# taaha-khan/2023-CompaCT-Image-Compression

Hardware: AMD Instinct MI355X
Metric: MPixels/s encode+decode, 12-bit 512x512 CT batch, bytes-exact (higher is better)
Workload: dtype u16

## Files before the change

2023-compact-image-compression_amd/csrc/deflate_kernels.hip:

```cpp
#include <hip/hip_runtime.h>
#include <cstring>
#include <algorithm>

#include "cct_internal.h"
#include "../../include/compact_hip.h"

namespace cct {
namespace {

constexpr int MIN_MATCH = 3, MAX_MATCH = 258, WSIZE = 32768;
constexpr int MIN_LOOKAHEAD = MAX_MATCH + MIN_MATCH + 1;
constexpr int MAX_DIST = WSIZE - MIN_LOOKAHEAD;
constexpr int TOO_FAR = 4096;
constexpr int BLOCK_SYMS = 16383;
constexpr int L_CODES = 286, D_CODES = 30, BL_CODES = 19, HEAP_SIZE = 2 * L_CODES + 1;
constexpr int END_BLOCK = 256, MAX_BITS = 15, MAX_BL_BITS = 7;

__constant__ uint8_t c_extra_lbits[29] = {0,0,0,0,0,0,0,0,1,1,1,1,2,2,2,2,3,3,3,3,4,4,4,4,5,5,5,5,0};
__constant__ uint8_t c_extra_dbits[30] = {0,0,0,0,1,1,2,2,3,3,4,4,5,5,6,6,7,7,8,8,9,9,10,10,11,11,12,12,13,13};
__constant__ uint8_t c_extra_blbits[19] = {0,0,0,0,0,0,0,0,0,0,0,0,0,0,0,0,2,3,7};
__constant__ uint8_t c_bl_order[19] = {16,17,18,0,8,7,9,6,10,5,11,4,12,3,13,2,14,1,15};
__constant__ uint8_t c_length_code[256];
__constant__ uint16_t c_base_length[29];
__constant__ uint8_t c_dist_code[512];
// ... 582 lines not shown
	uint32_t ie = base_es[0] + inc_e - ne, is = base_es[1] + inc_s - ns, tot_e = base_es[0];
	for (int w2 = 0; w2 < 4; w2++) {
		const uint32_t te = wsum_e[w2], ts = wsum_s[w2];
		if (w2 < wave) { ie += te; is += ts; }
		tot_e += te;
	}
	if ((uint32_t)tid * 8 < (uint32_t)RUNLEN_OUT && g < L) re[3 * (a.in_stride >> 2) + (g >> 3)] = ie;
#pragma unroll
	for (int k = 0; k < 8; k++) {
		if ((me >> k) & 1u) re[ie++] = g + k + 3;
		if ((ms >> k) & 1u) rs[is++] = g + k;
	}
	if (tid == 0 && c0 + RUNLEN_OUT >= L) a.run_end_count[s] = tot_e;
}

__global__ void __launch_bounds__(256) dfl_run_info_kernel(DeflateArgs a)
{
	const int s = blockIdx.y;
	const uint8_t *in = a.in + (size_t)s * a.in_stride;
	const uint32_t *re = a.run_ends + (size_t)s * a.in_stride;
	const uint32_t *rs = re + (a.in_stride >> 2);
	uint32_t *rl = a.run_ends + (size_t)s * a.in_stride + (a.in_stride >> 1);
	const uint32_t nre = a.run_end_count[s];
	for (uint32_t t = blockIdx.x * blockDim.x + threadIdx.x; t < nre; t += gridDim.x * blockDim.x) {
		const uint32_t x = re[t], len = x - rs[t];
		rl[t] = (len < 511u ? len : 511u) | ((uint32_t)in[x - 1] << 16);
	}
}

__global__ void __launch_bounds__(256) dfl_match_run_kernel(DeflateArgs a, int n)
{
	int s; uint32_t part, nparts;
	if (!xcd_slice(n, s, part, nparts)) return;
	const uint32_t L = a.in_sizes[s];
	const uint8_t *in = a.in + (size_t)s * a.in_stride;
	const size_t base = (size_t)s * a.in_stride;
	const uint64_t *recs = a.rec_out + base;
	uint2 *mr = reinterpret_cast<uint2 *>(a.mr) + base;
	const uint32_t *deep = a.heavy_list + base + a.in_stride - 1;
	const uint32_t ndeep = a.deep_count[s];
	const uint32_t *re = a.run_ends + base;
	const uint32_t *rl = re + (a.in_stride >> 1);
	const uint32_t nre = a.run_end_count[s];
	const uint32_t gen = *a.gen;
	for (uint32_t e = part * blockDim.x + threadIdx.x; e < ndeep; e += nparts * blockDim.x) {
		const uint32_t i = *(deep - e);
		const uint64_t ri = recs[i];
		const uint64_t r_head = recs[i >= 1 ? i - 1 : 0], r_1024 = recs[i >= 1024 ? i - 1024 : 0], r_4096 = recs[i >= 4096 ? i - 4096 : 0];
		const uint32_t p = rec_pos(ri, a.pos_mask);
		const uint32_t h = rec_hash(ri);
		const uint32_t lookahead = L - p;
		const uint32_t max_len = lookahead < (uint32_t)MAX_MATCH ? lookahead : (uint32_t)MAX_MATCH;
		const uint8_t b = in[p], b_prev = in[p >= 1 ? p - 1 : 0];
		const uint32_t r = a.run_len[base + p] & 0x7FFFu;
		const bool has_prev = p >= 2 && b_prev == b;
		uint32_t best4 = has_prev ? r : 0u, q4 = p - 1, best1 = best4, q1 = p - 1;
		bool scan = true;
		if (!has_prev) {
			const uint64_t rh = i >= 1 ? r_head : ~0ull;
			const bool have_head = i >= 1 && rec_hash(rh) == h;
			const uint32_t hq = have_head ? rec_pos(rh, a.pos_mask) : 0u;
			if (!have_head || hq == 0 || hq == nil_candidate(p, lookahead) || p - hq > (uint32_t)MAX_DIST) scan = false;
			else if (p - hq == (uint32_t)MAX_DIST) {
				uint32_t len = 0;
				len = (uint32_t)common_prefix(in + hq, in + p, 0, (int)max_len);
				best4 = best1 = len; q4 = q1 = hq;
				scan = false;
			}
		}
		if (scan && best4 < max_len) {
			const bool ext_ok = r < max_len;
			const uint8_t c = ext_ok ? in[p + r] : 0;
			const uint32_t qw = p >= (uint32_t)MAX_DIST ? p - (uint32_t)MAX_DIST + 1 : 1u;
			uint32_t qmin4 = qw, qmin1 = qw;
			if (i >= 4096 && rec_hash(r_4096) == h) qmin4 = max(qmin4, rec_pos(r_4096, a.pos_mask));
			if (i >= 1024 && rec_hash(r_1024) == h) qmin1 = max(qmin1, rec_pos(r_1024, a.pos_mask));
			uint32_t lo = 0;
			if (p >= 3) {
				lo = re[3 * (a.in_stride >> 2) + ((p - 2) >> 3)];
				while (lo < nre && re[lo] <= p) lo++;
			}
			uint32_t x_n = lo ? re[lo - 1] : 0u, lw_n = lo ? rl[lo - 1] : 0u;
			for (int64_t t = (int64_t)lo - 1; t >= 0; t--) {
				const uint32_t x = x_n;
				const uint32_t lw = lw_n;
				{ const int64_t tn = t > 0 ? t - 1 : 0; x_n = re[tn]; lw_n = rl[tn]; }
				if (x < qmin4 + 3) break;
				if ((lw >> 16) != b) continue;
				const uint32_t m = min(min(lw & 0xFFFFu, r), x - qmin4);
				if (m >= 3) {
					uint32_t q, len;
					if (m == r) {
						q = x - r; len = r;
						if (ext_ok && in[x] == c) len = (uint32_t)common_prefix(in + q, in + p, (int)r + 1, (int)max_len);
					} else { q = x - m; len = m; }
					if (len > best4) { best4 = len; q4 = q; }
					if (x >= qmin1 + 3) {
						const uint32_t m1 = min(m, x - qmin1);
						if (m1 == m) { if (len > best1) { best1 = len; q1 = q; } }
						else if (m1 >= 3 && m1 > best1) { best1 = m1; q1 = x - m1; }
					}
					if (best4 >= max_len) break;
				}
				if (x - m <= qmin4) break;
			}
		}
		mr[p] = pack_match(best4, best1, best4 ? p - q4 : 0u, best1 ? p - q1 : 0u, gen);
	}
}

__device__ __forceinline__ void match_of(const MatchRec &r, uint32_t p, uint32_t npos, int prev_len, int &len, int &dist)
{
	len = 2; dist = 0;
	if (p >= npos || prev_len >= MAX_MATCH) return;
	const int l = prev_len >= 32 ? r.len1024 : r.len4096;
	const int d = prev_len >= 32 ? r.dist1024 : r.dist4096;
	if (l > prev_len && l >= MIN_MATCH) { len = l; dist = d; }
	if (len == MIN_MATCH && dist > TOO_FAR) len = 2;
}
__device__ __forceinline__ void match_at(const MatchRec *mr, const uint16_t *rl, uint32_t gen, uint32_t p, uint32_t npos, int prev_len, int &len, int &dist)
{
	len = 2; dist = 0;
	if (p >= npos || prev_len >= MAX_MATCH) return;
	match_of(checked_match(mr[p], gen, rl[p], p, npos + 2), p, npos, prev_len, len, dist);
}

__global__ void __launch_bounds__(256) dfl_rec_kernel(DeflateArgs a)
{
	const int s = blockIdx.y;
	const uint32_t L = a.in_sizes[s];
	const size_t base = (size_t)s * a.in_stride;
	const uint32_t npos = L >= MIN_MATCH ? L - 2 : 0;
	const MatchRec *mr = reinterpret_cast<const MatchRec *>(a.mr) + base;
	const uint16_t *rl = a.run_len + base;
	const uint32_t nblk64 = (L + 63) / 64;
	const int lane = threadIdx.x & 63;
	const uint32_t gen = *a.gen;
	const uint32_t lastp = npos ? npos - 1 : 0;
	const uint32_t wb_step = gridDim.x * (blockDim.x >> 6);
	struct Req { MatchRec m0, m1; uint32_t w0, w1; };
	auto request = [&](uint32_t wb) {
		const uint32_t p = wb * 64 + lane, pa = min(p, lastp), pb = min(p + 1, lastp);
		return Req{mr[pa], mr[pb], rl[pa], rl[pb]};
	};
	const uint32_t wb0 = blockIdx.x * (blockDim.x >> 6) + (threadIdx.x >> 6);
	Req nx = request(wb0);
	for (uint32_t wb = wb0; wb < nblk64; wb += wb_step) {
		const uint32_t p = wb * 64 + lane;
		const uint32_t blk_end = wb * 64 + 64;
		uint32_t rec = 0, nxt = blk_end, cnt = 0;
		const uint32_t pa = min(p, lastp), pb = min(p + 1, lastp);
		const Req cq = nx;
		nx = request(wb + wb_step);
		const MatchRec r0 = checked_match(cq.m0, gen, cq.w0, pa, L), r1 = checked_match(cq.m1, gen, cq.w1, pb, L);
		if (p < L) {
			int len, dist;
			match_of(r0, p, npos, 2, len, dist);
			if (len < MIN_MATCH) { rec = 0; nxt = p + 1; cnt = 1; }
			else {
				uint32_t k = 0;
				for (;;) {
					int l2, d2;
					if (k == 0) match_of(r1, p + 1, npos, len, l2, d2);
					else match_at(mr, rl, gen, p + k + 1, npos, len, l2, d2);
					if (l2 > len) { len = l2; dist = d2; k++; } else break;
				}
				rec = k | ((uint32_t)len << 8) | ((uint32_t)dist << 17);
				nxt = p + k + (uint32_t)len;
				cnt = k + 1;
			}
		}
		a.rec32[base + p] = rec;
#pragma unroll
		for (int r = 0; r < 6; r++) {
			const bool inside = nxt < blk_end;
			const int j = inside ? (int)(nxt - wb * 64) : lane;
			const uint32_t n2 = __shfl(nxt, j), c2 = __shfl(cnt, j);
			if (inside) { nxt = n2; cnt += c2; }
		}
		a.exit_pos[base + p] = (nxt - blk_end) | (cnt << 16);
	}
}

#ifndef CCT_WALK_T
#define CCT_WALK_T 256
#endif
constexpr int WALK_T = CCT_WALK_T;
__global__ void __launch_bounds__(WALK_T) dfl_walk_kernel(DeflateArgs a, int n)
{
	__shared__ uint32_t s_land[WALK_T];
	__shared__ uint32_t s_wsum[WALK_T / 64];
	const int s = blockIdx.x;
	(void)n;
	const uint32_t L = a.in_sizes[s];
	const size_t base = (size_t)s * a.in_stride;
	const size_t bbase = (size_t)s * (a.in_stride / 64);
	const uint32_t *exit_rec = a.exit_pos + base;
	const int tid = threadIdx.x, lane = tid & 63, wave = tid >> 6;
	const uint32_t seg = (((L + WALK_T - 1) / WALK_T) + 63) & ~63u;
	const uint32_t seg_end = min(L, (uint32_t)(tid + 1) * seg);
	uint32_t start = min(L, (uint32_t)tid * seg), land = start, cnt = 0;
	auto hop_through = [&]() {
		uint32_t cur = start, c = 0;
		while (cur < seg_end) { const uint32_t e = exit_rec[cur]; c += e >> 16; cur = (cur & ~63u) + 64u + (e & 0xFFFFu); }
		land = cur; cnt = c;
	};
	hop_through();
	for (;;) {
		__syncthreads();
		s_land[tid] = land;
		__syncthreads();
		const uint32_t pl = tid ? s_land[tid - 1] : 0u;
		const bool moved = tid > 0 && pl != start;
		if (!__syncthreads_or(moved)) break;
		if (moved) { start = pl; hop_through(); }
	}
	uint32_t inc = cnt;
#pragma unroll
	for (int d = 1; d < 64; d <<= 1) { const uint32_t o = __shfl_up(inc, d, 64); if (lane >= d) inc += o; }
	if (lane == 63) s_wsum[wave] = inc;
	__syncthreads();
	uint32_t syms = inc - cnt;
	for (int w = 0; w < wave; w++) syms += s_wsum[w];
	if (tid == WALK_T - 1) a.total_syms[s] = syms + cnt;
	for (uint32_t cur = start; cur < seg_end;) {
		const uint32_t b = cur >> 6;
		a.blk_entry[bbase + b] = cur;
		a.blk_symbase[bbase + b] = syms;
		const uint32_t e = exit_rec[cur];
		syms += e >> 16;
		cur = (cur & ~63u) + 64u + (e & 0xFFFFu);
	}
}

__global__ void __launch_bounds__(256) dfl_symbols_kernel(DeflateArgs a)
{
	const int s = blockIdx.y;
	const uint32_t L = a.in_sizes[s];
	const uint8_t *in = a.in + (size_t)s * a.in_stride;
	const size_t base = (size_t)s * a.in_stride;
	const size_t bbase = (size_t)s * (a.in_stride / 64);
	const uint32_t nblk64 = (L + 63) / 64;
	const int lane = threadIdx.x & 63;
	uint32_t *sym = a.sym + base;
	uint32_t *bend = a.blk_end + (size_t)s * a.max_blocks;
	const uint32_t wb_step = gridDim.x * (blockDim.x >> 6), wb_last = nblk64 ? nblk64 - 1 : 0;
	struct Req { uint32_t entry, symbase, rec; uint8_t lit0; };
	auto request = [&](uint32_t wb) {
		const uint32_t wbc = min(wb, wb_last), pc = min(wbc * 64 + lane, L - 1);
		return Req{a.blk_entry[bbase + wbc], a.blk_symbase[bbase + wbc], a.rec32[base + pc], in[pc]};
	};
	const uint32_t wb0 = blockIdx.x * (blockDim.x >> 6) + (threadIdx.x >> 6);
	Req nx = nblk64 ? request(wb0) : Req{0xFFFFFFFFu, 0, 0, 0};
	for (uint32_t wb = wb0; wb < nblk64; wb += wb_step) {
		const uint32_t p = wb * 64 + lane;
		const Req cur_req = nx;
		nx = request(wb + wb_step);
		const uint32_t entry = cur_req.entry, symbase = cur_req.symbase;
		uint32_t rec = cur_req.rec;
		const uint8_t lit0 = cur_req.lit0;
		if (entry == 0xFFFFFFFFu) continue;
		if (p >= L) rec = 0;
		const uint32_t k = rec & 0xFFu, len = (rec >> 8) & 0x1FFu, dist = rec >> 17;
		const uint32_t nxt = len ? p + k + len : p + 1;
		const uint32_t cnt = len ? k + 1 : 1;
		const uint64_t jump = __ballot(len != 0);
		const uint32_t nvalid = min(64u, L - wb * 64);
		uint64_t visited = 0;
		uint32_t cur = (uint32_t)__builtin_amdgcn_readfirstlane((int)(entry - wb * 64));
		while (cur < nvalid) {
			const uint64_t rest = jump >> cur;
			if (!rest) { visited |= ~0ull << cur; break; }
			const int d = __ffsll((long long)rest) - 1;
			visited |= (d >= 63 ? ~0ull : ((2ull << d) - 1ull)) << cur;
			cur = (uint32_t)__builtin_amdgcn_readlane((int)nxt, (int)cur + d) - wb * 64;
		}
		if (nvalid < 64) visited &= (1ull << nvalid) - 1ull;
		const bool mine = (visited >> lane) & 1ull;
		uint32_t v = mine ? cnt : 0u, inc = v;
#pragma unroll
		for (int d = 1; d < 64; d <<= 1) {
			const uint32_t t = __shfl_up(inc, d);
			if (lane >= d) inc += t;
		}
		uint32_t off = symbase + inc - v;
		if (mine) {
			if (p == L - 1) a.postloop_lit[s] = 1;
			for (uint32_t t = 0; t < (len ? k : 1u); t++, off++) {
				sym[off] = t ? in[p + t] : lit0;
				if (off % BLOCK_SYMS == BLOCK_SYMS - 1) bend[off / BLOCK_SYMS] = p + t + 1;
			}
			if (len) {
				sym[off] = (len - MIN_MATCH) | (dist << 16);
				if (off % BLOCK_SYMS == BLOCK_SYMS - 1) bend[off / BLOCK_SYMS] = p + k + len;
			}
		}
	}
}

struct TreeScratch {
	uint16_t freq[HEAP_SIZE], dad[HEAP_SIZE], len[HEAP_SIZE], code[L_CODES + 2];
	uint16_t dfreq[2 * D_CODES + 1], ddad[2 * D_CODES + 1], dlen[2 * D_CODES + 1], dcode[D_CODES + 2];
	uint16_t bfreq[2 * BL_CODES + 1], bdad[2 * BL_CODES + 1], blen[2 * BL_CODES + 1], bcode[BL_CODES + 1];
	alignas(16) uint32_t heap[HEAP_SIZE + 3];
	uint32_t bl_count[MAX_BITS + 1];
	uint16_t next_code[MAX_BITS + 1];
	int heap_len, heap_max, max_code, overflow, lmax, dmax;
	uint32_t opt_len, static_len, dyn_body_bits;
	uint32_t hdr_bits[160];
	uint32_t hdr_nbits;
	int ntok, btype, max_blindex;
	uint8_t extra_l[29], extra_d[30], extra_bl[19], bl_order[19];
	__device__ __forceinline__ uint32_t *hist_l() { return heap; }
	__device__ __forceinline__ uint32_t *hist_d() { return heap + L_CODES + 2; }
	__device__ __forceinline__ uint8_t *length_code() { return reinterpret_cast<uint8_t *>(dad); }
	__device__ __forceinline__ uint8_t *dist_code() { return reinterpret_cast<uint8_t *>(dad) + 256; }
	__device__ __forceinline__ uint16_t *tok() { return dad; }
};
static_assert(sizeof(TreeScratch) <= 8192, "13 tree waves per CU: keep the working set around 8 KB");
static_assert(HEAP_SIZE >= L_CODES + D_CODES, "token list fits dad[]");
static_assert((HEAP_SIZE + 1) * 4 >= (L_CODES + 2 + D_CODES) * 4 && HEAP_SIZE * 2 >= 768, "aliases fit");
__device__ __forceinline__ uint32_t static_llen(int n) { return n <= 143 ? 8u : n <= 255 ? 9u : n <= 279 ? 7u : 8u; }

typedef __attribute__((address_space(3))) uint16_t lds_u16;
struct TreeView { lds_u16 *freq, *dad, *len, *code; };

__device__ __forceinline__ uint32_t uni(uint32_t x) { return (uint32_t)__builtin_amdgcn_readfirstlane((int)x); }
__device__ __forceinline__ void pqdownheap(TreeScratch &S, int k, int hl)
{
	const uint32_t v = uni(S.heap[k]);
	const uint32_t vk = v >> 10;
	int j = k << 1;
	while (j <= hl) {
		uint2 pr = *reinterpret_cast<const uint2 *>(&S.heap[j]);
		uint4 gc = *reinterpret_cast<const uint4 *>(&S.heap[min(2 * j, (HEAP_SIZE & ~3))]);
		pr.x = uni(pr.x); pr.y = uni(pr.y);
		gc.x = uni(gc.x); gc.y = uni(gc.y); gc.z = uni(gc.z); gc.w = uni(gc.w);
		uint32_t e = pr.x;
		int c = j;
		if (j < hl && (pr.y >> 10) <= (pr.x >> 10)) { c = j + 1; e = pr.y; }
		if (vk <= (e >> 10)) break;
		S.heap[k] = e;
		k = c;
		j = c << 1;
		if (j > hl) break;
		const bool left = (c & 1) == 0;
		const uint32_t x2 = left ? gc.x : gc.z, y2 = left ? gc.y : gc.w;
		e = x2;
		c = j;
		if (j < hl && (y2 >> 10) <= (x2 >> 10)) { c = j + 1; e = y2; }
		if (vk <= (e >> 10)) break;
		S.heap[k] = e;
		k = c;
		j = c << 1;
	}
	S.heap[k] = v;
}

__device__ __forceinline__ uint32_t sift_root(TreeScratch &S, uint32_t v, int hl, int levels)
{
	if (levels == 0) { S.heap[1] = v; return v; }
	const uint2 p0 = *reinterpret_cast<const uint2 *>(&S.heap[2]);
	uint32_t right = (2 < hl && p0.y <= (p0.x | 1023u)) ? 1u : 0u;
	uint32_t e = right ? p0.y : p0.x;
	uint32_t moving = v > (e | 1023u) ? 1u : 0u;
	const uint32_t rootv = moving ? e : v;
	S.heap[1] = rootv;
	uint32_t k = 2u + right;
	for (int l = 1; l < levels - 1; l++) {
		const uint32_t j = k << 1;
		const uint2 pr = *reinterpret_cast<const uint2 *>(&S.heap[j]);
		right = pr.y <= (pr.x | 1023u) ? 1u : 0u;
		e = right ? pr.y : pr.x;
		const uint32_t go = (moving && v > (e | 1023u)) ? 1u : 0u;
		S.heap[moving ? k : 0u] = go ? e : v;
		k = go ? j + right : k;
		moving = go;
	}
	if (levels >= 2) {
		const uint32_t j = k << 1;
		const uint2 pr = *reinterpret_cast<const uint2 *>(&S.heap[min(j, (uint32_t)(HEAP_SIZE - 1))]);
		right = (j < (uint32_t)hl && pr.y <= (pr.x | 1023u)) ? 1u : 0u;
		e = right ? pr.y : pr.x;
		const uint32_t go = (moving && j <= (uint32_t)hl && v > (e | 1023u)) ? 1u : 0u;
		S.heap[moving ? k : 0u] = go ? e : v;
		k = go ? j + right : k;
		moving = go;
	}
	S.heap[moving ? k : 0u] = v;
	return rootv;
}


__device__ __forceinline__ TreeView view_of(TreeScratch &S, int kind)
{
	if (kind == 0) return TreeView{(lds_u16 *)S.freq, (lds_u16 *)S.dad, (lds_u16 *)S.len, (lds_u16 *)S.code};
	if (kind == 1) return TreeView{(lds_u16 *)S.dfreq, (lds_u16 *)S.ddad, (lds_u16 *)S.dlen, (lds_u16 *)S.dcode};
	return TreeView{(lds_u16 *)S.bfreq, (lds_u16 *)S.bdad, (lds_u16 *)S.blen, (lds_u16 *)S.bcode};
}
__device__ __forceinline__ int elems_of(int kind) { return kind == 0 ? L_CODES : kind == 1 ? D_CODES : BL_CODES; }

__device__ void tree_leaves(TreeScratch &S, int kind)
{
	const TreeView t = view_of(S, kind);
	const int lane = threadIdx.x, elems = elems_of(kind);
	const uint64_t lt_mask = (1ull << lane) - 1ull;
	int max_code = -1;
	uint32_t nleaf = 0;
	for (int n0 = 0; n0 < elems; n0 += 64) {
		const int n = n0 + lane;
		const uint32_t f = n < elems ? t.freq[n] : 0u;
		const uint64_t bal = __ballot(f != 0);
		if (f != 0) S.heap[1 + nleaf + (uint32_t)__popcll(bal & lt_mask)] = (f << 15) | (uint32_t)n;
		else if (n < elems) t.len[n] = 0;
		if (bal) max_code = n0 + 63 - __clzll((long long)bal);
		nleaf += (uint32_t)__popcll(bal);
	}
	if (lane == 0) { S.heap_len = (int)nleaf; S.max_code = max_code; }
}

__device__ void tree_heap(TreeScratch &S, int kind)
{
	const TreeView t = view_of(S, kind);
	int n, m, node, max_code = (int)uni((uint32_t)S.max_code);
	int heap_len = (int)uni((uint32_t)S.heap_len), heap_max = HEAP_SIZE;
	while (heap_len < 2) {
		node = max_code < 2 ? ++max_code : 0;
		t.freq[node] = 1; S.opt_len--;
		S.heap[++heap_len] = (1u << 15) | (uint32_t)node;
		if (kind == 0) S.static_len -= static_llen(node);
		else if (kind == 1) S.static_len -= 5;
	}
	for (n = heap_len / 2; n >= 1; n--) pqdownheap(S, n, heap_len);
	node = elems_of(kind);
	uint32_t top = S.heap[1];
	do {
		const uint32_t en = top;
		const uint32_t lastv = S.heap[heap_len];
		heap_len--;
		const int levels = 31 - __clz(heap_len | 1);
		const uint32_t em = sift_root(S, lastv, heap_len, levels);
		n = (int)(en & 1023u); m = (int)(em & 1023u);
		S.heap[--heap_max] = en; S.heap[--heap_max] = em;
		const uint32_t f = (en >> 15) + (em >> 15);
		const uint32_t dn = (en >> 10) & 31u, dm = (em >> 10) & 31u;
		const uint32_t d = (dn >= dm ? dn : dm) + 1;
		t.freq[node] = (uint16_t)f;
		t.dad[n] = t.dad[m] = (uint16_t)node;
		top = sift_root(S, (f << 15) | (d << 10) | (uint32_t)node, heap_len, levels);
		node++;
	} while (heap_len >= 2);
	S.heap[--heap_max] = top;
	S.heap_len = heap_len; S.heap_max = heap_max;
	S.max_code = max_code;
}

__device__ void tree_depths(TreeScratch &S, int kind)
{
	const TreeView t = view_of(S, kind);
	const int lane = threadIdx.x;
	const int max_length = kind == 2 ? MAX_BL_BITS : MAX_BITS;
	const int base = kind == 0 ? 257 : 0;
	const int max_code = S.max_code, heap_max = S.heap_max;
	const uint32_t root = S.heap[heap_max];
	constexpr uint16_t UNKNOWN = 0xFFFF;
	for (int h = heap_max + 1 + lane; h < HEAP_SIZE; h += 64) t.len[S.heap[h] & 1023u] = UNKNOWN;
	if (lane == 0) t.len[root & 1023u] = 0;
	if (lane <= MAX_BITS) S.bl_count[lane] = 0;
	__syncthreads();
	for (bool again = true; again;) {
		again = false;
		for (int h0 = heap_max + 1; h0 < HEAP_SIZE; h0 += 64) {
			const int h = h0 + lane;
			bool unknown = false;
			if (h < HEAP_SIZE) {
				const int n = (int)(S.heap[h] & 1023u);
				if (t.len[n] == UNKNOWN) {
					const uint32_t ld = t.len[t.dad[n]];
					if (ld == UNKNOWN) unknown = true;
					else t.len[n] = (uint16_t)min(ld + 1u, (uint32_t)max_length);
				}
			}
			if (__ballot(unknown)) again = true;
		}
		__syncthreads();
	}
	int overflow = 0;
	for (int h0 = heap_max + 1; h0 < HEAP_SIZE; h0 += 64) {
		const int h = h0 + lane;
		const bool clamped = h < HEAP_SIZE && t.len[t.dad[S.heap[h] & 1023u]] == (uint32_t)max_length;
		overflow += (int)__popcll(__ballot(clamped));
	}
	uint32_t o = 0, st = 0;
	for (int n = lane; n <= max_code; n += 64) {
		const uint32_t f = t.freq[n];
		if (f == 0) continue;
		const uint32_t bits = t.len[n];
		atomicAdd(&S.bl_count[bits], 1u);
		uint32_t xbits = 0;
		if (n >= base) xbits = kind == 0 ? S.extra_l[n - base] : kind == 1 ? S.extra_d[n] : S.extra_bl[n];
		o += f * (bits + xbits);
		if (kind == 0) st += f * (static_llen(n) + xbits);
		else if (kind == 1) st += f * (5u + xbits);
	}
	o = wave_sum(o); st = wave_sum(st);
	if (lane == 0) { S.overflow = overflow; S.opt_len += o; S.static_len += st; }
}

__device__ void tree_fix(TreeScratch &S, int kind)
{
	const TreeView t = view_of(S, kind);
	const int max_length = kind == 2 ? MAX_BL_BITS : MAX_BITS;
	const int max_code = S.max_code;
	int overflow = S.overflow;
	if (overflow > 0) {
		int bits, n, m, h = HEAP_SIZE;
		do {
			bits = max_length - 1;
			while (S.bl_count[bits] == 0) bits--;
			S.bl_count[bits]--; S.bl_count[bits + 1] += 2; S.bl_count[max_length]--;
			overflow -= 2;
		} while (overflow > 0);
		for (bits = max_length; bits != 0; bits--) {
			n = (int)S.bl_count[bits];
			while (n != 0) {
				m = (int)(S.heap[--h] & 1023u);
				if (m > max_code) continue;
				if ((uint32_t)t.len[m] != (uint32_t)bits) {
					S.opt_len += ((uint32_t)bits - t.len[m]) * t.freq[m];
					t.len[m] = (uint16_t)bits;
				}
				n--;
			}
		}
	}
	uint32_t code = 0;
	for (int bits = 1; bits <= MAX_BITS; bits++) { code = (code + S.bl_count[bits - 1]) << 1; S.next_code[bits] = (uint16_t)code; }
}

__device__ void tree_codes(TreeScratch &S, int kind)
{
	const TreeView t = view_of(S, kind);
	const int lane = threadIdx.x, max_code = S.max_code;
	const uint64_t lt_mask = (1ull << lane) - 1ull;
	uint32_t seen[MAX_BITS + 1];
#pragma unroll
	for (int b = 1; b <= MAX_BITS; b++) seen[b] = S.next_code[b];
	for (int n0 = 0; n0 <= max_code; n0 += 64) {
		const int n = n0 + lane;
		const int len = n <= max_code ? (int)t.len[n] : 0;
		uint32_t mine = 0;
#pragma unroll
		for (int b = 1; b <= MAX_BITS; b++) {
			const uint64_t bal = __ballot(len == b);
			if (len == b) mine = seen[b] + (uint32_t)__popcll(bal & lt_mask);
			seen[b] += (uint32_t)__popcll(bal);
		}
		if (len != 0) t.code[n] = (uint16_t)(__brev(mine) >> (32 - len));
	}
}

__device__ void scan_tree_wave(TreeScratch &S, const TreeView &t, int max_code)
{
	const int lane = threadIdx.x;
	constexpr int NCH = (L_CODES + 63) / 64;
	const int n_el = max_code + 1;
	uint32_t v[NCH];
	uint64_t startmask[NCH];
#pragma unroll
	for (int c = 0; c < NCH; c++) {
		const int n = c * 64 + lane;
		v[c] = n < n_el ? (uint32_t)t.len[n] : 0xFFFFu;
		const uint32_t before = n == 0 ? 0xFFFFFFFFu : (uint32_t)t.len[max(n - 1, 0)];
		startmask[c] = __ballot(n < n_el && v[c] != before);
	}
	uint16_t *tk = S.tok();
	uint32_t base = (uint32_t)S.ntok;
#pragma unroll
	for (int c = 0; c < NCH; c++) {
		if (c * 64 >= n_el) break;
		const int n = c * 64 + lane;
		const bool start = (startmask[c] >> lane) & 1ull;
		uint32_t R = 0;
		if (start) {
			int nxt = n_el;
			const uint64_t rest = lane < 63 ? startmask[c] >> (lane + 1) : 0ull;
			if (rest) nxt = n + (int)__ffsll((long long)rest);
			else {
#pragma unroll
				for (int c2 = NCH - 1; c2 > c; c2--) if (startmask[c2]) nxt = min(nxt, c2 * 64 + (int)__ffsll((long long)startmask[c2]) - 1);
			}
			R = (uint32_t)(nxt - n);
		}
		const uint32_t val = v[c];
		uint32_t nlit_head = 0, nrep6 = 0, tail_lit = 0, tail_sym = 0xFFFFFFFFu, nbig = 0;
		if (start) {
			if (val != 0) {
				if (R < 4) nlit_head = R;
				else if (R <= 6) { nlit_head = 1; tail_sym = 16u | ((R - 4u) << 5); }
				else {
					nlit_head = 1; nrep6 = 1 + (R - 7u) / 6u;
					const uint32_t r = (R - 7u) % 6u;
					if (r < 3) tail_lit = r; else tail_sym = 16u | ((r - 3u) << 5);
				}
			} else {
				nbig = R / 138u;
				const uint32_t r = R % 138u;
				if (r < 3) tail_lit = r;
				else if (r <= 10) tail_sym = 17u | ((r - 3u) << 5);
				else tail_sym = 18u | ((r - 11u) << 5);
			}
		}
		const uint32_t ntok = nlit_head + nrep6 + nbig + tail_lit + (tail_sym != 0xFFFFFFFFu ? 1u : 0u);
		uint32_t inc = ntok;
#pragma unroll
		for (int d = 1; d < 64; d <<= 1) { const uint32_t o = (uint32_t)__shfl_up((int)inc, d, 64); if (lane >= d) inc += o; }
		if (start) {
			uint32_t w = base + inc - ntok;
			for (uint32_t i = 0; i < nlit_head; i++) tk[w++] = (uint16_t)val;
			for (uint32_t i = 0; i < nrep6; i++) tk[w++] = (uint16_t)(16u | (3u << 5));
			for (uint32_t i = 0; i < nbig; i++) tk[w++] = (uint16_t)(18u | (127u << 5));
			for (uint32_t i = 0; i < tail_lit; i++) tk[w++] = (uint16_t)val;
			if (tail_sym != 0xFFFFFFFFu) tk[w++] = (uint16_t)tail_sym;
			if (nlit_head + tail_lit) atomicAdd(&S.hdr_bits[val], nlit_head + tail_lit);
			if (nrep6) atomicAdd(&S.hdr_bits[16], nrep6);
			if (nbig) atomicAdd(&S.hdr_bits[18], nbig);
			if (tail_sym != 0xFFFFFFFFu) atomicAdd(&S.hdr_bits[tail_sym & 31u], 1u);
		}
		base += (uint32_t)__shfl((int)inc, 63, 64);
	}
	if (lane == 0) S.ntok = (int)base;
}

__device__ __forceinline__ void hdr_or(TreeScratch &S, uint32_t pos, uint32_t value, uint32_t n)
{
	const uint32_t w = pos >> 5, sh = pos & 31u;
	atomicOr(&S.hdr_bits[w], value << sh);
	if (sh + n > 32u) atomicOr(&S.hdr_bits[w + 1], value >> (32u - sh));
}

__device__ void send_header(TreeScratch &S)
{
	const int lane = threadIdx.x;
	const int nbl = S.max_blindex + 1;
	if (lane == 0) hdr_or(S, 0, (uint32_t)(S.lmax + 1 - 257) | ((uint32_t)(S.dmax + 1 - 1) << 5) | ((uint32_t)(nbl - 4) << 10), 14);
	if (lane < nbl) hdr_or(S, 14u + 3u * (uint32_t)lane, S.blen[S.bl_order[lane]], 3);
	uint32_t base = 14u + 3u * (uint32_t)nbl;
	const uint16_t *tk = S.tok();
	const int nt = S.ntok;
	for (int c0 = 0; c0 < nt; c0 += 64) {
		const int i = c0 + lane;
		uint32_t nbits = 0, val = 0;
		if (i < nt) {
			const uint32_t sym = tk[i] & 31u, ex = tk[i] >> 5;
			const uint32_t cl = S.blen[sym];
			nbits = cl + S.extra_bl[sym];
			val = (uint32_t)S.bcode[sym] | (ex << cl);
		}
		uint32_t inc = nbits;
#pragma unroll
		for (int d = 1; d < 64; d <<= 1) { const uint32_t o = (uint32_t)__shfl_up((int)inc, d, 64); if (lane >= d) inc += o; }
		if (nbits) hdr_or(S, base + inc - nbits, val, nbits);
		base += (uint32_t)__shfl((int)inc, 63, 64);
	}
	if (lane == 0) S.hdr_nbits = base;
}

constexpr int TREE_BLOCKS = 1;
__global__ void __launch_bounds__(64) dfl_tree_kernel(DeflateArgs a)
{
	__shared__ TreeScratch S4[TREE_BLOCKS];
	const int s = blockIdx.y, m0 = blockIdx.x * TREE_BLOCKS, lane = threadIdx.x;
	const uint32_t T = a.total_syms[s];
	const uint32_t L = a.in_sizes[s];
	uint32_t nfull = T / BLOCK_SYMS;
	if (T % BLOCK_SYMS == 0 && nfull > 0 && a.postloop_lit[s]) nfull--;
	const uint32_t nblocks = nfull + 1;
	BlockMeta *meta = a.block_meta + (size_t)s * a.max_blocks;
	if ((uint32_t)m0 >= nblocks) return;
	const int nb = (int)min((uint32_t)TREE_BLOCKS, nblocks - (uint32_t)m0);
	const uint32_t *bend = a.blk_end + (size_t)s * a.max_blocks;
	const bool owner = lane < nb;
#ifdef CCT_TREE_PROF
	long long tp[16]; int tpi = 0;
#define TREE_STAMP() do { if (tpi < 16) tp[tpi++] = clock64(); } while (0)
#else
#define TREE_STAMP() do {} while (0)
#endif
	TREE_STAMP();

	for (int q = 0; q < nb; q++) {
		TreeScratch &S = S4[q];
		const int m = m0 + q;
		const bool last = (uint32_t)m == nblocks - 1;
		const uint32_t first = (uint32_t)m * BLOCK_SYMS;
		const uint32_t nsym = last ? T - first : (uint32_t)BLOCK_SYMS;
		const uint32_t *sym = a.sym + (size_t)s * a.in_stride + first;
		for (int i = lane; i < HEAP_SIZE; i += 64) { S.freq[i] = 0; S.len[i] = 0; }
		for (int i = lane; i < L_CODES + 2; i += 64) S.code[i] = 0;
		for (int i = lane; i < 2 * D_CODES + 1; i += 64) { S.dfreq[i] = 0; S.dlen[i] = 0; S.ddad[i] = 0; }
		for (int i = lane; i < D_CODES + 2; i += 64) S.dcode[i] = 0;
		for (int i = lane; i < 2 * BL_CODES + 1; i += 64) { S.bfreq[i] = 0; S.blen[i] = 0; S.bdad[i] = 0; }
		for (int i = lane; i < BL_CODES + 1; i += 64) S.bcode[i] = 0;
		uint8_t *length_code = S.length_code(), *dist_code = S.dist_code();
		{
			uint8_t dc[8], lc4[4];
#pragma unroll
			for (int k = 0; k < 8; k++) dc[k] = c_dist_code[lane + 64 * k];
#pragma unroll
			for (int k = 0; k < 4; k++) lc4[k] = c_length_code[lane + 64 * k];
			const int l29 = min(lane, 28), l30 = min(lane, 29), l19 = min(lane, 18);
			const uint8_t xl = c_extra_lbits[l29], xd = c_extra_dbits[l30], xb = c_extra_blbits[l19], bo = c_bl_order[l19];
#pragma unroll
			for (int k = 0; k < 8; k++) dist_code[lane + 64 * k] = dc[k];
#pragma unroll
			for (int k = 0; k < 4; k++) length_code[lane + 64 * k] = lc4[k];
			if (lane < 29) S.extra_l[lane] = xl;
			if (lane < 30) S.extra_d[lane] = xd;
			if (lane < 19) { S.extra_bl[lane] = xb; S.bl_order[lane] = bo; }
		}
		uint32_t *hl = S.hist_l(), *hd = S.hist_d();
		for (int i = lane; i < L_CODES; i += 64) hl[i] = 0;
		if (lane < D_CODES) hd[lane] = 0;
		__syncthreads();
		{
			const uint32_t lasts = nsym ? nsym - 1 : 0;
			uint32_t nv[16];
#pragma unroll
			for (int k = 0; k < 16; k++) nv[k] = sym[min((uint32_t)(k * 64 + lane), lasts)];
			for (uint32_t i0 = 0; i0 < nsym; i0 += 64 * 16) {
				uint32_t v[16];
#pragma unroll
				for (int k = 0; k < 16; k++) v[k] = nv[k];
#pragma unroll
				for (int k = 0; k < 16; k++) nv[k] = sym[min(i0 + 1024u + (uint32_t)(k * 64 + lane), lasts)];
#pragma unroll
				for (int k = 0; k < 16; k++) {
					if (i0 + (uint32_t)(k * 64 + lane) >= nsym) continue;
					const uint32_t dist = v[k] >> 16, lc = v[k] & 0xFFu;
					if (dist == 0) atomicAdd(&hl[lc], 1u);
					else {
						const uint32_t d1 = dist - 1;
						atomicAdd(&hl[length_code[lc] + 256 + 1], 1u);
						atomicAdd(&hd[d1 < 256 ? dist_code[d1] : dist_code[256 + (d1 >> 7)]], 1u);
					}
				}
			}
		}
		__syncthreads();
		for (int i = lane; i < L_CODES; i += 64) S.freq[i] = (uint16_t)hl[i];
		if (lane < D_CODES) S.dfreq[lane] = (uint16_t)hd[lane];
		for (int i = lane; i < 160; i += 64) S.hdr_bits[i] = 0;
		if (lane == 0) { S.opt_len = 0; S.static_len = 0; S.hdr_nbits = 0; S.ntok = 0; S.btype = 0; S.max_blindex = 0; }
		__syncthreads();
		if (lane == 0) S.freq[END_BLOCK] = 1;
		for (int i = lane; i < HEAP_SIZE; i += 64) S.dad[i] = 0;
	}
	__syncthreads();
	TREE_STAMP();
#pragma unroll 1
	for (int kind = 0; kind < 3; kind++) {
		if (kind == 2) {
			if (owner) S4[lane].dyn_body_bits = S4[lane].opt_len;
			__syncthreads();
			for (int q = 0; q < nb; q++) {
				TreeScratch &S = S4[q];
				scan_tree_wave(S, view_of(S, 0), S.lmax);
				__syncthreads();
				scan_tree_wave(S, view_of(S, 1), S.dmax);
				__syncthreads();
				if (lane < BL_CODES) { S.bfreq[lane] = (uint16_t)S.hdr_bits[lane]; S.hdr_bits[lane] = 0; }
			}
			__syncthreads();
		}
		for (int q = 0; q < nb; q++) tree_leaves(S4[q], kind);
		__syncthreads();
		TREE_STAMP();
		if (owner) tree_heap(S4[lane], kind);
		__syncthreads();
		TREE_STAMP();
		for (int q = 0; q < nb; q++) tree_depths(S4[q], kind);
		__syncthreads();
		if (owner) {
			tree_fix(S4[lane], kind);
			if (kind == 0) S4[lane].lmax = S4[lane].max_code; else if (kind == 1) S4[lane].dmax = S4[lane].max_code;
		}
		__syncthreads();
		for (int q = 0; q < nb; q++) tree_codes(S4[q], kind);
		__syncthreads();
		TREE_STAMP();
	}
	if (owner) {
		TreeScratch &S = S4[lane];
		const int m = m0 + lane;
		const bool last = (uint32_t)m == nblocks - 1;
		const uint32_t first = (uint32_t)m * BLOCK_SYMS;
		const uint32_t nsym = last ? T - first : (uint32_t)BLOCK_SYMS;
		const uint32_t in_begin = m == 0 ? 0u : bend[m - 1];
		const uint32_t in_end = last ? L : bend[m];
		int max_blindex;
		for (max_blindex = BL_CODES - 1; max_blindex >= 3; max_blindex--)
			if (S.blen[S.bl_order[max_blindex]] != 0) break;
		S.opt_len += 3 * ((uint32_t)max_blindex + 1) + 5 + 5 + 4;
		uint32_t opt_lenb = (S.opt_len + 3 + 7) >> 3;
		const uint32_t static_lenb = (S.static_len + 3 + 7) >> 3;
		if (static_lenb <= opt_lenb) opt_lenb = static_lenb;
		const uint32_t stored_len = in_end - in_begin;
		BlockMeta bm;
		bm.in_begin = in_begin; bm.stored_len = stored_len; bm.first_sym = first; bm.nsym = nsym; bm.last = last ? 1u : 0u;
		if (stored_len + 4 <= opt_lenb) {
			bm.type = 0; bm.hdr_nbits = 0; bm.body_bits = 0;
		} else if (static_lenb == opt_lenb) {
			bm.type = 1; bm.hdr_nbits = 0; bm.body_bits = S.static_len;
		} else {
			bm.type = 2; bm.hdr_nbits = 0;
			bm.body_bits = S.dyn_body_bits;
		}
		S.btype = (int)bm.type; S.max_blindex = max_blindex;
		meta[m] = bm;
		if (m == 0) a.n_blocks[s] = nblocks;
	}
	__syncthreads();
	for (int q = 0; q < nb; q++) {
		TreeScratch &S = S4[q];
		if (S.btype != 2) continue;
		send_header(S);
		__syncthreads();
		BlockTables *bt = a.block_tables + ((size_t)s * a.max_blocks + m0 + q);
		for (int i = lane; i * 32 < (int)S.hdr_nbits; i += 64) bt->hdr_bits[i] = S.hdr_bits[i];
		if (lane == 0) meta[m0 + q].hdr_nbits = S.hdr_nbits;
	}
	__syncthreads();
	TREE_STAMP();
#ifdef CCT_TREE_PROF
	if (s == 0 && m0 == 0 && lane == 0) {
		printf("[tree prof] nb=%d:", nb);
		for (int i = 1; i < tpi; i++) printf(" %lld", tp[i] - tp[i - 1]);
		printf("  (hist | leaves0 heap0 rest0 | scan+leaves1 heap1 rest1 | scan_tree+leaves2 heap2 rest2 | final)\n");
	}
#endif
	for (int q = 0; q < nb; q++) {
		TreeScratch &S = S4[q];
		BlockTables *bt = a.block_tables + ((size_t)s * a.max_blocks + m0 + q);
		for (int i = lane; i < L_CODES; i += 64) { bt->lcode[i] = S.code[i]; bt->llen[i] = (uint8_t)S.len[i]; }
		if (lane < D_CODES) { bt->dcode[lane] = S.dcode[lane]; bt->dlen[lane] = (uint8_t)S.dlen[lane]; }
	}
}

__global__ void __launch_bounds__(256) dfl_adler_kernel(DeflateArgs a)
{
	__shared__ unsigned long long sa[256], sb[256];
	const int s = blockIdx.x;
	const uint32_t L = a.in_sizes[s];
	const uint8_t *in = a.in + (size_t)s * a.in_stride;
	unsigned long long A = 0, B = 0;
	const uint32_t nfull = L / 16;
	constexpr int U = 8;
	for (uint32_t g0 = threadIdx.x; g0 < nfull; g0 += blockDim.x * U) {
		uint4 v[U];
#pragma unroll
		for (int u = 0; u < U; u++) v[u] = *reinterpret_cast<const uint4 *>(in + (size_t)min(g0 + (uint32_t)u * blockDim.x, nfull - 1) * 16);
#pragma unroll
		for (int u = 0; u < U; u++) {
			const uint32_t g = g0 + (uint32_t)u * blockDim.x;
			if (g >= nfull) continue;
			const uint32_t w[4] = {v[u].x, v[u].y, v[u].z, v[u].w};
			uint32_t sd = 0, sk = 0;
#pragma unroll
			for (int k = 0; k < 16; k++) { const uint32_t d = (w[k >> 2] >> ((k & 3) * 8)) & 0xFFu; sd += d; sk += (uint32_t)k * d; }
			A += sd;
			B += (unsigned long long)(L - g * 16) * sd - sk;
		}
	}
	if (threadIdx.x == 0)
		for (uint32_t i = nfull * 16; i < L; i++) { const unsigned long long d = in[i]; A += d; B += (unsigned long long)(L - i) * d; }
	sa[threadIdx.x] = A; sb[threadIdx.x] = B;
	__syncthreads();
	for (int st = 128; st > 0; st >>= 1) {
		if ((int)threadIdx.x < st) { sa[threadIdx.x] += sa[threadIdx.x + st]; sb[threadIdx.x] += sb[threadIdx.x + st]; }
		__syncthreads();
	}
	if (threadIdx.x == 0) {
		const uint32_t lo = (uint32_t)((1ull + sa[0]) % 65521ull);
		const uint32_t hi = (uint32_t)(((unsigned long long)L + sb[0]) % 65521ull);
		a.adler[s] = (hi << 16) | lo;
	}
}

__global__ void dfl_layout_kernel(DeflateArgs a, int n)
{
	const int s = blockIdx.x * blockDim.x + threadIdx.x;
	if (s >= n) return;
	uint8_t *out = a.out + (size_t)s * a.out_stride;
	for (int i = 0; i < 13; i++) out[i] = a.header13[i];
	out[13] = 0x78; out[14] = 0xDA;
	uint64_t bit = 8ull * 15;
	BlockMeta *meta = a.block_meta + (size_t)s * a.max_blocks;
	const uint32_t nb = a.n_blocks[s];
	for (uint32_t m = 0; m < nb; m++) {
		BlockMeta bm = meta[m];
		bm.bit_off = bit;
		if (bm.type == 0) {
			bit = (bit + 3 + 7) & ~7ull;
			bit += 32 + 8ull * bm.stored_len;
		} else {
			bit += 3 + bm.hdr_nbits + bm.body_bits;
		}
		if (bm.last) bit = (bit + 7) & ~7ull;
		meta[m] = bm;
	}
	const uint64_t byte = bit >> 3;
	const uint32_t ad = a.adler[s];
	out[byte + 0] = (uint8_t)(ad >> 24); out[byte + 1] = (uint8_t)(ad >> 16);
	out[byte + 2] = (uint8_t)(ad >> 8);  out[byte + 3] = (uint8_t)ad;
	a.out_sizes[s] = (uint32_t)(byte + 4);
}

__device__ __forceinline__ void or_bits(uint32_t *words, uint64_t bit, uint64_t value, int nbits)
{
	if (nbits == 0) return;
	const uint64_t w = bit >> 5;
	const int sh = (int)(bit & 31);
	const uint64_t lo = value << sh;
	const uint64_t hi = sh ? (value >> (64 - sh)) : 0ull;
	atomicOr(&words[w], (uint32_t)lo);
	if (sh + nbits > 32) atomicOr(&words[w + 1], (uint32_t)(lo >> 32));
	if (sh + nbits > 64) atomicOr(&words[w + 2], (uint32_t)hi);
}

__global__ void __launch_bounds__(256) dfl_emit_kernel(DeflateArgs a)
{
	__shared__ uint32_t wsum[4];
	__shared__ unsigned long long s_run;
	const int s = blockIdx.y, m = blockIdx.x;
	if ((uint32_t)m >= a.n_blocks[s]) return;
	const BlockMeta bm = a.block_meta[(size_t)s * a.max_blocks + m];
	const BlockTables *bt = a.block_tables + ((size_t)s * a.max_blocks + m);
	uint8_t *out = a.out + (size_t)s * a.out_stride;
	uint32_t *words = reinterpret_cast<uint32_t *>(out);
	const uint8_t *in = a.in + (size_t)s * a.in_stride;
	uint64_t bit = bm.bit_off;
	if (bm.type == 0) {
		if (threadIdx.x == 0) or_bits(words, bit, (uint64_t)bm.last, 3);
		const uint64_t byte = ((bit + 3 + 7) & ~7ull) >> 3;
		if (threadIdx.x == 0) {
			out[byte] = (uint8_t)(bm.stored_len & 0xFF); out[byte + 1] = (uint8_t)(bm.stored_len >> 8);
			out[byte + 2] = (uint8_t)(~bm.stored_len & 0xFF); out[byte + 3] = (uint8_t)((~bm.stored_len >> 8) & 0xFF);
		}
		for (uint32_t i = threadIdx.x; i < bm.stored_len; i += blockDim.x) out[byte + 4 + i] = in[bm.in_begin + i];
		return;
	}
	if (threadIdx.x == 0) or_bits(words, bit, (uint64_t)((bm.type << 1) + bm.last), 3);
	bit += 3;
	if (bm.type == 2) {
		for (uint32_t i = threadIdx.x; i * 32 < bm.hdr_nbits; i += blockDim.x) {
			const int nb = (int)min(32u, bm.hdr_nbits - i * 32);
			or_bits(words, bit + 32ull * i, bt->hdr_bits[i], nb);
		}
		bit += bm.hdr_nbits;
	}
	const uint32_t *sym = a.sym + (size_t)s * a.in_stride + bm.first_sym;
	const bool dyn = bm.type == 2;
	const int lane = threadIdx.x & 63, wave = threadIdx.x >> 6;
	__shared__ uint16_t t_lcode[L_CODES + 2], t_dcode[D_CODES + 2];
	__shared__ uint8_t t_llen[L_CODES + 2], t_dlen[D_CODES + 2];
	__shared__ uint32_t wbuf[400];
	__shared__ uint8_t t_length_code[256], t_dist_code[512], t_extra_l[32], t_extra_d[32];
	__shared__ uint16_t t_base_length[32], t_base_dist[32];
	{
		const int t = threadIdx.x, t2 = min(t + 256, L_CODES - 1), td = min(t, D_CODES - 1), t29 = min(t, 28), t30 = min(t, 29);
		const uint16_t *lsrc = dyn ? bt->lcode : c_static_lcode, *dsrc = dyn ? bt->dcode : c_static_dcode;
		const uint8_t *llsrc = dyn ? bt->llen : c_static_llen;
		const uint16_t lc0 = lsrc[t], lc1 = lsrc[t2];
		const uint8_t ll0 = llsrc[t], ll1 = llsrc[t2];
		const uint16_t dc = dsrc[td];
		uint8_t dl = bt->dlen[td];
		if (!dyn) dl = 5;
		const uint8_t k0 = c_dist_code[t], k1 = c_dist_code[t + 256], lcd = c_length_code[t];
		const uint8_t xl = c_extra_lbits[t29], xd = c_extra_dbits[t30];
		const uint16_t bl = c_base_length[t29], bd = c_base_dist[t30];
		t_lcode[t] = lc0; t_llen[t] = ll0;
		if (t + 256 < L_CODES) { t_lcode[t + 256] = lc1; t_llen[t + 256] = ll1; }
		if (t < D_CODES) { t_dcode[t] = dc; t_dlen[t] = dl; }
		t_dist_code[t] = k0; t_dist_code[t + 256] = k1; t_length_code[t] = lcd;
		if (t < 29) { t_extra_l[t] = xl; t_base_length[t] = bl; }
		if (t < 30) { t_extra_d[t] = xd; t_base_dist[t] = bd; }
	}
	if (threadIdx.x == 0) s_run = bit;
	for (int i = threadIdx.x; i < 400; i += blockDim.x) wbuf[i] = 0;
	__syncthreads();
	const uint32_t last_sym = bm.nsym ? bm.nsym - 1 : 0;
	uint32_t vnext = sym[min((uint32_t)threadIdx.x, last_sym)];
	for (uint32_t base = 0; base <= bm.nsym; base += blockDim.x) {
		const uint32_t i = base + threadIdx.x;
		uint64_t bits = 0;
		int nb = 0;
		const uint32_t v = vnext;
		vnext = sym[min(i + blockDim.x, last_sym)];
		if (i < bm.nsym) {
			uint32_t dist = v >> 16;
			const uint32_t lc = v & 0xFFu;
			if (dist == 0) {
				bits = t_lcode[lc];
				nb = t_llen[lc];
			} else {
				int code = t_length_code[lc];
				const int lsym = code + 256 + 1;
				bits = t_lcode[lsym];
				nb = t_llen[lsym];
				int extra = t_extra_l[code];
				if (extra) { bits |= (uint64_t)(lc - t_base_length[code]) << nb; nb += extra; }
				dist--;
				code = dist < 256 ? t_dist_code[dist] : t_dist_code[256 + (dist >> 7)];
				bits |= (uint64_t)t_dcode[code] << nb;
				nb += t_dlen[code];
				extra = t_extra_d[code];
				if (extra) { bits |= (uint64_t)(dist - t_base_dist[code]) << nb; nb += extra; }
			}
		} else if (i == bm.nsym) {
			bits = t_lcode[END_BLOCK];
			nb = t_llen[END_BLOCK];
		}
		uint32_t inc = (uint32_t)nb;
#pragma unroll
		for (int d = 1; d < 64; d <<= 1) {
			const uint32_t t = __shfl_up(inc, d);
			if (lane >= d) inc += t;
		}
		if (lane == 63) wsum[wave] = inc;
		__syncthreads();
		uint32_t wb = 0, tot = 0;
		for (int w = 0; w < 4; w++) { if (w < wave) wb += wsum[w]; tot += wsum[w]; }
		const uint64_t run = s_run;
		const uint32_t lbit = (uint32_t)(run & 31) + wb + inc - (uint32_t)nb;
		if (nb) {
			const uint32_t w0 = lbit >> 5, sh = lbit & 31;
			const uint64_t lo = bits << sh;
			atomicOr(&wbuf[w0], (uint32_t)lo);
			if (sh + nb > 32) atomicOr(&wbuf[w0 + 1], (uint32_t)(lo >> 32));
			if (sh + nb > 64) atomicOr(&wbuf[w0 + 2], (uint32_t)(bits >> (64 - sh)));
		}
		__syncthreads();
		const uint32_t nwords = ((uint32_t)(run & 31) + tot + 31) >> 5;
		const uint64_t gw = run >> 5;
		for (uint32_t k = threadIdx.x; k < nwords; k += blockDim.x) {
			const uint32_t v = wbuf[k];
			if (v) atomicOr(&words[gw + k], v);
			wbuf[k] = 0;
		}
		if (threadIdx.x == 0) s_run = run + tot;
		__syncthreads();
	}
}

__global__ void __launch_bounds__(256) dfl_pack_offsets_kernel(const uint32_t *sizes, int n, uint64_t *offsets, int exact)
{
	if (threadIdx.x == 0 && blockIdx.x == 0) {
		uint64_t acc = 0;
		for (int i = 0; i < n; i++) { offsets[i] = acc; acc += exact ? sizes[i] : ((sizes[i] + 15u) & ~15u); }
		offsets[n] = acc;
	}
}
__global__ void __launch_bounds__(256) dfl_pack_kernel(const uint8_t *src, size_t stride, const uint32_t *sizes,
                                                       const uint64_t *offsets, uint8_t *dst)
{
	const int s = blockIdx.y;
	const uint32_t n16 = (sizes[s] + 15u) >> 4;
	const uint4 *in = reinterpret_cast<const uint4 *>(src + (size_t)s * stride);
	uint4 *out = reinterpret_cast<uint4 *>(dst + offsets[s]);
	for (uint32_t i = blockIdx.x * blockDim.x + threadIdx.x; i < n16; i += gridDim.x * blockDim.x) out[i] = in[i];
}

__global__ void dfl_offsets2_kernel(DeflateArgs a, int n)
{
	const size_t per = a.in_stride / 64;
	for (size_t i = blockIdx.x * (size_t)blockDim.x + threadIdx.x; i < (size_t)n * per; i += (size_t)gridDim.x * blockDim.x)
		a.blk_entry[i] = 0xFFFFFFFFu;
}

__global__ void dfl_offsets_kernel(DeflateArgs a, int n)
{
// ... 129 lines not shown
```

Before: 15470.

## Pipeline Huffman heap sifts across wave lanes instead of one lane per block

Huffman tree construction changes from one lane handling a whole block to a whole wave cooperating on each block in turn. Heapify now runs level by level with lanes sifting nodes in parallel, and the extract/merge loop keeps up to eight sift-downs in flight on separate lanes. Each sift advances one level per tick and a ballot checks for conflicts before the next pop. This targets the long serial dependency chain of the heap loop, but blocks are now processed one after another rather than one per lane, and the lane-synchronised ticking adds overhead and correctness risk.

Result: faster. 16240 (median of 6 runs) (+5.0%).

```diff
diff --git a/2023-compact-image-compression_amd/csrc/deflate_kernels.hip b/2023-compact-image-compression_amd/csrc/deflate_kernels.hip
--- a/2023-compact-image-compression_amd/csrc/deflate_kernels.hip
+++ b/2023-compact-image-compression_amd/csrc/deflate_kernels.hip
@@ -908,7 +908,7 @@
 	uint16_t freq[HEAP_SIZE], dad[HEAP_SIZE], len[HEAP_SIZE], code[L_CODES + 2];
 	uint16_t dfreq[2 * D_CODES + 1], ddad[2 * D_CODES + 1], dlen[2 * D_CODES + 1], dcode[D_CODES + 2];
 	uint16_t bfreq[2 * BL_CODES + 1], bdad[2 * BL_CODES + 1], blen[2 * BL_CODES + 1], bcode[BL_CODES + 1];
-	alignas(16) uint32_t heap[HEAP_SIZE + 3];
+	alignas(16) uint32_t heap[HEAP_SIZE + 11];
 	uint32_t bl_count[MAX_BITS + 1];
 	uint16_t next_code[MAX_BITS + 1];
 	int heap_len, heap_max, max_code, overflow, lmax, dmax;
@@ -931,72 +931,19 @@
 typedef __attribute__((address_space(3))) uint16_t lds_u16;
 struct TreeView { lds_u16 *freq, *dad, *len, *code; };
 
-__device__ __forceinline__ uint32_t uni(uint32_t x) { return (uint32_t)__builtin_amdgcn_readfirstlane((int)x); }
 __device__ __forceinline__ void pqdownheap(TreeScratch &S, int k, int hl)
 {
-	const uint32_t v = uni(S.heap[k]);
-	const uint32_t vk = v >> 10;
-	int j = k << 1;
-	while (j <= hl) {
-		uint2 pr = *reinterpret_cast<const uint2 *>(&S.heap[j]);
-		uint4 gc = *reinterpret_cast<const uint4 *>(&S.heap[min(2 * j, (HEAP_SIZE & ~3))]);
-		pr.x = uni(pr.x); pr.y = uni(pr.y);
-		gc.x = uni(gc.x); gc.y = uni(gc.y); gc.z = uni(gc.z); gc.w = uni(gc.w);
-		uint32_t e = pr.x;
-		int c = j;
-		if (j < hl && (pr.y >> 10) <= (pr.x >> 10)) { c = j + 1; e = pr.y; }
-		if (vk <= (e >> 10)) break;
+	const uint32_t v = S.heap[k];
+	for (int j = k << 1; j <= hl; j = k << 1) {
+		const uint2 pr = *reinterpret_cast<const uint2 *>(&S.heap[j]);
+		const int right = (j < hl && pr.y <= (pr.x | 1023u)) ? 1 : 0;
+		const uint32_t e = right ? pr.y : pr.x;
+		if (v <= (e | 1023u)) break;
 		S.heap[k] = e;
-		k = c;
-		j = c << 1;
-		if (j > hl) break;
-		const bool left = (c & 1) == 0;
-		const uint32_t x2 = left ? gc.x : gc.z, y2 = left ? gc.y : gc.w;
-		e = x2;
-		c = j;
-		if (j < hl && (y2 >> 10) <= (x2 >> 10)) { c = j + 1; e = y2; }
-		if (vk <= (e >> 10)) break;
-		S.heap[k] = e;
-		k = c;
-		j = c << 1;
+		k = j + right;
 	}
 	S.heap[k] = v;
 }
-
-__device__ __forceinline__ uint32_t sift_root(TreeScratch &S, uint32_t v, int hl, int levels)
-{
-	if (levels == 0) { S.heap[1] = v; return v; }
-	const uint2 p0 = *reinterpret_cast<const uint2 *>(&S.heap[2]);
-	uint32_t right = (2 < hl && p0.y <= (p0.x | 1023u)) ? 1u : 0u;
-	uint32_t e = right ? p0.y : p0.x;
-	uint32_t moving = v > (e | 1023u) ? 1u : 0u;
-	const uint32_t rootv = moving ? e : v;
-	S.heap[1] = rootv;
-	uint32_t k = 2u + right;
-	for (int l = 1; l < levels - 1; l++) {
-		const uint32_t j = k << 1;
-		const uint2 pr = *reinterpret_cast<const uint2 *>(&S.heap[j]);
-		right = pr.y <= (pr.x | 1023u) ? 1u : 0u;
-		e = right ? pr.y : pr.x;
-		const uint32_t go = (moving && v > (e | 1023u)) ? 1u : 0u;
-		S.heap[moving ? k : 0u] = go ? e : v;
-		k = go ? j + right : k;
-		moving = go;
-	}
-	if (levels >= 2) {
-		const uint32_t j = k << 1;
-		const uint2 pr = *reinterpret_cast<const uint2 *>(&S.heap[min(j, (uint32_t)(HEAP_SIZE - 1))]);
-		right = (j < (uint32_t)hl && pr.y <= (pr.x | 1023u)) ? 1u : 0u;
-		e = right ? pr.y : pr.x;
-		const uint32_t go = (moving && j <= (uint32_t)hl && v > (e | 1023u)) ? 1u : 0u;
-		S.heap[moving ? k : 0u] = go ? e : v;
-		k = go ? j + right : k;
-		moving = go;
-	}
-	S.heap[moving ? k : 0u] = v;
-	return rootv;
-}
-
 
 __device__ __forceinline__ TreeView view_of(TreeScratch &S, int kind)
 {
@@ -1025,40 +972,86 @@
 	if (lane == 0) { S.heap_len = (int)nleaf; S.max_code = max_code; }
 }
 
+constexpr int TREE_SIFTS = 8;
 __device__ void tree_heap(TreeScratch &S, int kind)
 {
 	const TreeView t = view_of(S, kind);
-	int n, m, node, max_code = (int)uni((uint32_t)S.max_code);
-	int heap_len = (int)uni((uint32_t)S.heap_len), heap_max = HEAP_SIZE;
-	while (heap_len < 2) {
-		node = max_code < 2 ? ++max_code : 0;
-		t.freq[node] = 1; S.opt_len--;
-		S.heap[++heap_len] = (1u << 15) | (uint32_t)node;
-		if (kind == 0) S.static_len -= static_llen(node);
-		else if (kind == 1) S.static_len -= 5;
-	}
-	for (n = heap_len / 2; n >= 1; n--) pqdownheap(S, n, heap_len);
-	node = elems_of(kind);
-	uint32_t top = S.heap[1];
-	do {
-		const uint32_t en = top;
-		const uint32_t lastv = S.heap[heap_len];
-		heap_len--;
-		const int levels = 31 - __clz(heap_len | 1);
-		const uint32_t em = sift_root(S, lastv, heap_len, levels);
-		n = (int)(en & 1023u); m = (int)(em & 1023u);
-		S.heap[--heap_max] = en; S.heap[--heap_max] = em;
-		const uint32_t f = (en >> 15) + (em >> 15);
-		const uint32_t dn = (en >> 10) & 31u, dm = (em >> 10) & 31u;
-		const uint32_t d = (dn >= dm ? dn : dm) + 1;
-		t.freq[node] = (uint16_t)f;
-		t.dad[n] = t.dad[m] = (uint16_t)node;
-		top = sift_root(S, (f << 15) | (d << 10) | (uint32_t)node, heap_len, levels);
-		node++;
-	} while (heap_len >= 2);
-	S.heap[--heap_max] = top;
-	S.heap_len = heap_len; S.heap_max = heap_max;
-	S.max_code = max_code;
+	const int lane = threadIdx.x;
+	int max_code = S.max_code, h = S.heap_len;
+	while (h < 2) {
+		const int node = max_code < 2 ? ++max_code : 0;
+		h++;
+		if (lane == 0) {
+			t.freq[node] = 1; S.opt_len--;
+			S.heap[h] = (1u << 15) | (uint32_t)node;
+			if (kind == 0) S.static_len -= static_llen(node);
+			else if (kind == 1) S.static_len -= 5;
+		}
+	}
+	__syncthreads();
+	for (int d = 31 - __clz(h >> 1); d >= 0; d--) {
+		const int lo = 1 << d, hi = min((2 << d) - 1, h >> 1);
+		for (int n0 = lo; n0 <= hi; n0 += 64) {
+			if (n0 + lane <= hi) pqdownheap(S, n0 + lane, h);
+			__builtin_amdgcn_wave_barrier();
+		}
+	}
+	if (lane < TREE_SIFTS) {
+		uint32_t v = 0, k = 1, hl = 0, w = 0;
+		bool moving = false;
+		const uint32_t sink = HEAP_SIZE + 3 + lane;
+		auto tick = [&]() {
+			const uint32_t j = k << 1;
+			const uint2 pr = *reinterpret_cast<const uint2 *>(&S.heap[j]);
+			const uint32_t right = (j < hl && pr.y <= (pr.x | 1023u)) ? 1u : 0u;
+			const uint32_t e = right ? pr.y : pr.x;
+			const bool go = moving && j <= hl && v > (e | 1023u);
+			w = go ? e : v;
+			uint32_t at = moving ? k : sink;
+			asm volatile("" : "+v"(at), "+v"(w));
+			S.heap[at] = w;
+			k = go ? j + right : k;
+			moving = go;
+			__builtin_amdgcn_wave_barrier();
+		};
+		auto start = [&](int slot, uint32_t x) {
+			const bool me = lane == slot;
+			v = me ? x : v; k = me ? 1u : k; hl = me ? (uint32_t)h : hl; moving = moving || me;
+		};
+		int node = elems_of(kind), hm = HEAP_SIZE, slot = 0;
+		uint32_t en = S.heap[1];
+		for (;;) {
+			while (__ballot(moving && ((uint32_t)h >> (__clz(k | 1u) - __clz(h))) == k)) tick();
+			h--;
+			start(slot, S.heap[h + 1]);
+			tick();
+			const uint32_t em = (uint32_t)__builtin_amdgcn_readlane((int)w, slot);
+			const uint32_t f = (en >> 15) + (em >> 15);
+			const uint32_t dn = (en >> 10) & 31u, dm = (em >> 10) & 31u;
+			const uint32_t d = (dn >= dm ? dn : dm) + 1;
+			if (lane == 0) {
+				S.heap[hm - 1] = en; S.heap[hm - 2] = em;
+				t.freq[node] = (uint16_t)f;
+				t.dad[en & 1023u] = t.dad[em & 1023u] = (uint16_t)node;
+			}
+			hm -= 2;
+			slot = (slot + 1) & (TREE_SIFTS - 1);
+			tick();
+			start(slot, (f << 15) | (d << 10) | (uint32_t)node);
+			tick();
+			en = (uint32_t)__builtin_amdgcn_readlane((int)w, slot);
+			slot = (slot + 1) & (TREE_SIFTS - 1);
+			node++;
+			if (h < 2) break;
+			tick();
+		}
+		while (__ballot(moving)) tick();
+		if (lane == 0) {
+			S.heap[--hm] = en;
+			S.heap_len = h; S.heap_max = hm;
+			S.max_code = max_code;
+		}
+	}
 }
 
 __device__ void tree_depths(TreeScratch &S, int kind)
@@ -1382,7 +1375,7 @@
 		for (int q = 0; q < nb; q++) tree_leaves(S4[q], kind);
 		__syncthreads();
 		TREE_STAMP();
-		if (owner) tree_heap(S4[lane], kind);
+		for (int q = 0; q < nb; q++) tree_heap(S4[q], kind);
 		__syncthreads();
 		TREE_STAMP();
 		for (int q = 0; q < nb; q++) tree_depths(S4[q], kind);
```
